# nickirk/pymes

Measured on AMD Instinct MI355X. Metric: ccsd_iteration_time, lower is better.
Workload: dtype f64

## Files before the change

include/pymes_amd.h:

```cpp
#ifndef PYMES_AMD_H
#define PYMES_AMD_H

#include <stdint.h>

#ifdef __cplusplus
extern "C" {
#endif

typedef struct pymes_ctx pymes_ctx;

#define PYMES_NOCC_MAX_FUSED 90
#define PYMES_NOCC_MAX_LAMBDA 88
#define PYMES_NOCC_MAX_BRA_DRESS 80

const char* pymes_last_error(void);
const char* pymes_backend(void);
int pymes_ctx_create(pymes_ctx** out, int device, int no, int nv, uint64_t workspace_bytes );
int pymes_ctx_destroy(pymes_ctx* ctx);
int pymes_ctx_set_stream(pymes_ctx* ctx, void* hip_stream);
int pymes_ctx_sync(pymes_ctx* ctx);
int pymes_ctx_workspace(pymes_ctx* ctx, uint64_t* capacity_bytes, uint64_t* high_water_bytes);

int pymes_malloc(pymes_ctx* ctx, uint64_t bytes, void** dev_ptr);
int pymes_free(pymes_ctx* ctx, void* dev_ptr);
// ... 14 lines not shown
int pymes_download(pymes_ctx* ctx, void* dst_host, const void* src_dev, uint64_t bytes);
int pymes_copy(pymes_ctx* ctx, void* dst_dev, const void* src_dev, uint64_t bytes);
int pymes_memset_zero(pymes_ctx* ctx, void* dst_dev, uint64_t bytes);

int pymes_contract(pymes_ctx* ctx, double alpha,
                   const double* A_dev, const char* la, const int64_t* dimA, const int64_t* strideA,
                   const double* B_dev, const char* lb, const int64_t* dimB, const int64_t* strideB,
                   double beta, double* C_dev, const char* lc, const int64_t* dimC, const int64_t* strideC,
                   const char* batch);
int pymes_permute(pymes_ctx* ctx, double alpha, const double* in_dev, const char* li, const int64_t* dim_in,
                  const int64_t* stride_in, double beta, double* out_dev, const char* lo,
                  const int64_t* stride_out);
int pymes_dgemm(pymes_ctx* ctx, int64_t M, int64_t N, int64_t K, double alpha, const double* A_dev, int64_t a_sm,
                int64_t a_sk, const double* B_dev, int64_t b_sk, int64_t b_sn, double beta, double* C_dev,
                int64_t ldc);

int pymes_set_V_pqrs(pymes_ctx* ctx, const double* V, int on_device, const int64_t* strides);
int pymes_set_V_block(pymes_ctx* ctx, const char* name, const double* data, int64_t n_elements, int on_device,
                      const int64_t* strides);
int pymes_V_exchange_asymmetry(pymes_ctx* ctx, double* out_host);
int pymes_exchange_asymmetry(pymes_ctx* ctx, const double* A_dev, const double* B_dev, const int64_t* dims,
                             double* out_host);
int pymes_set_V_from_factors(pymes_ctx* ctx, const double* B_host, int naux);
int pymes_set_integral_shard(pymes_ctx* ctx, int rank, int world);
int pymes_set_integral_direct(pymes_ctx* ctx, int64_t chunk_bytes);
int pymes_direct_info(pymes_ctx* ctx, int64_t* info);
int pymes_direct_rows(pymes_ctx* ctx, int64_t r0, int64_t r1, const double** vp, const double** vm, int64_t* ldp, int64_t* ldm);
int pymes_integral_bytes(pymes_ctx* ctx, int64_t* bytes);
int pymes_shard_rows_ptr(pymes_ctx* ctx, const double** vp, const double** vm, int64_t* row0, int64_t* row1, int64_t* ldp,
                         int64_t* ldm);
// ... 299 lines not shown
```

pymes_amd/_lib.py:

```python
import ctypes as C
import os

import numpy as np

_HERE = os.path.dirname(os.path.abspath(__file__))
DEFAULT_PATH = os.environ.get("PYMES_AMD_LIBRARY") or os.path.join(_HERE, "lib", "libpymes_amd.so")

c_double_p = C.POINTER(C.c_double)
c_i64_p = C.POINTER(C.c_int64)


class ShardBuffers(C.Structure):
    _fields_ = [(k, C.c_void_p) for k in ("ETd", "ETx", "L", "QK", "Tall", "W", "Xvv", "P", "R1", "S")]

c_pp = C.POINTER(C.c_void_p)

RESPONSE_HIST = 32
RESPONSE_DOTS = 2 * (RESPONSE_HIST + 2)


class ResponseSystem(C.Structure):
    _fields_ = ([(k, C.c_void_p * 2) for k in ("x", "r", "p", "ap", "pn")]
                + [(k, (C.c_void_p * 2) * RESPONSE_HIST) for k in ("hp", "hq")]
                + [("g", (C.c_double * 2) * RESPONSE_HIST), ("alpha", C.c_double * 2), ("z", C.c_double * 2), ("inv", C.c_double),
# ... 20 lines not shown
    "pymes_graph_abort": (C.c_int, [C.c_void_p]),
    "pymes_graph_launch": (C.c_int, [C.c_void_p, C.c_void_p]),
    "pymes_graph_destroy": (C.c_int, [C.c_void_p, C.c_void_p]),
    "pymes_upload": (C.c_int, [C.c_void_p, C.c_void_p, C.c_void_p, C.c_uint64]),
    "pymes_download": (C.c_int, [C.c_void_p, C.c_void_p, C.c_void_p, C.c_uint64]),
    "pymes_copy": (C.c_int, [C.c_void_p, C.c_void_p, C.c_void_p, C.c_uint64]),
    "pymes_memset_zero": (C.c_int, [C.c_void_p, C.c_void_p, C.c_uint64]),
    "pymes_contract": (C.c_int, [C.c_void_p, C.c_double,
                                 C.c_void_p, C.c_char_p, c_i64_p, c_i64_p,
                                 C.c_void_p, C.c_char_p, c_i64_p, c_i64_p,
                                 C.c_double, C.c_void_p, C.c_char_p, c_i64_p, c_i64_p, C.c_char_p]),
    "pymes_permute": (C.c_int, [C.c_void_p, C.c_double, C.c_void_p, C.c_char_p, c_i64_p, c_i64_p,
                                C.c_double, C.c_void_p, C.c_char_p, c_i64_p]),
    "pymes_dgemm": (C.c_int, [C.c_void_p, C.c_int64, C.c_int64, C.c_int64, C.c_double, C.c_void_p, C.c_int64,
                              C.c_int64, C.c_void_p, C.c_int64, C.c_int64, C.c_double, C.c_void_p, C.c_int64]),
    "pymes_set_V_pqrs": (C.c_int, [C.c_void_p, C.c_void_p, C.c_int, c_i64_p]),
    "pymes_set_V_block": (C.c_int, [C.c_void_p, C.c_char_p, C.c_void_p, C.c_int64, C.c_int, c_i64_p]),
    "pymes_V_exchange_asymmetry": (C.c_int, [C.c_void_p, c_double_p]),
    "pymes_exchange_asymmetry": (C.c_int, [C.c_void_p, C.c_void_p, C.c_void_p, c_i64_p, c_double_p]),
    "pymes_set_V_from_factors": (C.c_int, [C.c_void_p, C.c_void_p, C.c_int]),
    "pymes_V_block_ptr": (C.c_int, [C.c_void_p, C.c_char_p, C.c_int, c_pp, c_i64_p]),
    "pymes_set_integral_shard": (C.c_int, [C.c_void_p, C.c_int, C.c_int]),
    "pymes_integral_bytes": (C.c_int, [C.c_void_p, c_i64_p]),
    "pymes_set_integral_direct": (C.c_int, [C.c_void_p, C.c_int64]),
    "pymes_direct_info": (C.c_int, [C.c_void_p, c_i64_p]),
    "pymes_direct_rows": (C.c_int, [C.c_void_p, C.c_int64, C.c_int64, c_pp, c_pp, c_i64_p, c_i64_p]),
    "pymes_shard_rows_ptr": (C.c_int, [C.c_void_p, c_pp, c_pp, c_i64_p, c_i64_p, c_i64_p, c_i64_p]),
    "pymes_ccsd_t_triples": (C.c_int, [C.c_void_p, c_i64_p]),
    "pymes_ccsd_t": (C.c_int, [C.c_void_p, C.c_void_p, C.c_void_p, C.c_void_p, C.c_int64, C.c_int64, C.c_void_p,
                               c_double_p]),
# ... 215 lines not shown
```

pymes_amd/csrc/capi.cpp:

```cpp
#include <chrono>
#include <cstdio>
#include <cstring>
#include <exception>
#include <algorithm>
#include <mutex>
#include <set>
#include <string>
#include <vector>

#include "../../include/pymes_amd.h"
#include "diis_small.h"
#include "engine.h"
#include "eom.h"
#include "fcidump.h"
#include "packed.h"

using pymes::Engine;
using pymes::TView;

struct pymes_ctx {
    Engine* e;
};
struct pymes_eom {
    pymes::EomSigma* s;
// ... 238 lines not shown
        if (static_cast<int>(std::strlen(lo)) != r) throw pymes::Error("permute: label strings differ in length");
        int64_t dout[6];
        for (int i = 0; i < r; ++i) {
            const char* f = std::strchr(li, lo[i]);
            if (!f) throw pymes::Error("permute: output label missing from input");
            dout[i] = dim_in[f - li];
        }
        need_forward(stride_out, r, "stride_out");
        TView vout = pymes::make_view(out, r, dout, stride_out);
        need(out, "out");
        E(ctx).permute(alpha, vin, li, beta, vout, lo);
    });
}
int pymes_dgemm(pymes_ctx* ctx, int64_t M, int64_t N, int64_t K, double alpha, const double* A, int64_t a_sm,
                int64_t a_sk, const double* B, int64_t b_sk, int64_t b_sn, double beta, double* C, int64_t ldc) {
    return guarded([&] {
        Engine& e = Eq(ctx);
        dev::Gemm g{};
        g.M = M; g.N = N; g.K = K; g.alpha = alpha; g.beta = beta;
        g.A = A; g.a_sm = a_sm; g.a_sk = a_sk;
        g.B = B; g.b_sk = b_sk; g.b_sn = b_sn;
        g.C = C; g.ldc = ldc;
        g.nb1 = g.nb2 = 1;
        g.splitk_ws = e.splitk_ws();
        g.splitk_ws_doubles = e.splitk_ws_doubles();
        dev::gemm(g, e.stream);
        e.stats.gemm_calls++;
        e.stats.gemm_flops += 2.0 * double(M) * double(N) * double(K);
    });
}

int pymes_set_V_pqrs(pymes_ctx* ctx, const double* V, int on_device, const int64_t* strides) {
    return guarded([&] {
        need(V, "V");
        if (on_device) need_forward(strides, 4, "strides");
        E(ctx).set_V_full(V, on_device != 0, strides);
    });
// ... 1280 lines not shown
```

pymes_amd/csrc/kernels.hip:

```cpp
#include <hip/hip_runtime.h>
#include <type_traits>

#include <algorithm>
#include <atomic>
#include <chrono>
#include <cmath>
#include <cstdio>
#include <cstdlib>
#include <cstring>
#include <mutex>
#include <stdexcept>
#include <string>
#include <vector>

#include "../../include/pymes_amd.h"
#include "device_api.h"
#include "diis_small.h"
#include "device_util.h"
#include "launch.h"

namespace {

constexpr int kThreads = 256;
constexpr int BK = 16;
// ... 3 lines not shown
    const double* B;
    double* C;
    const double* Cin;
    long a_ld, b_ld, ldc;
    int M, N, K;
    int Mc, Nc;
    double alpha, beta;
    int tiles_m, tiles_n;
    int nsplit, kchunk;
    long tile_begin;
    long nb2;
    long a_b1, a_b2, b_b1, b_b2, c_b1, c_b2;
    double* ws;
    long whole = 0, tail = 0;
    int mixed = 0;
};

__device__ __forceinline__ long xcd_remap(long b, long nblk) {
    const long q = nblk >> 3, r = nblk & 7;
    const long xcd = b & 7, pos = b >> 3;
    return (xcd < r ? xcd * (q + 1) : r * (q + 1) + (xcd - r) * q) + pos;
}

template <int BM, int BN, bool AKC, bool BKC, int VEC, bool STREAM = false>
__device__ __forceinline__ void dgemm_body(const GemmK& g, const long bid) {
    extern __shared__ __attribute__((aligned(16))) double smem[];
    constexpr int WM = BM / 2, WN = BN / 2;
    constexpr int FM = WM / 16, FN = WN / 16;
    constexpr int A_PITCH = AKC ? (BK + 2) : (BM + 16);
    constexpr int A_ROWS = AKC ? BM : BK;
    constexpr int A_TILE = A_PITCH * A_ROWS;
    constexpr int B_PITCH = BKC ? (BK + 2) : (BN + 16);
    constexpr int B_ROWS = BKC ? BN : BK;
    constexpr int B_TILE = B_PITCH * B_ROWS;
    constexpr int LA = BM * BK / (kThreads * VEC);
    constexpr int LB = BN * BK / (kThreads * VEC);
// ... 291 lines not shown
    const unsigned lo = __builtin_amdgcn_readfirstlane((unsigned)v);
    const unsigned hi = __builtin_amdgcn_readfirstlane((unsigned)(v >> 32));
    return (const char*)(((unsigned long long)hi << 32) | lo);
}

__device__ __forceinline__ void glds16_su(const char* base_uniform, unsigned voff, unsigned lds_addr_uniform) {
    asm volatile("s_mov_b32 m0, %2\n\ts_nop 0\n\tglobal_load_lds_dwordx4 %0, %1"
                 :
                 : "v"(voff), "s"(base_uniform), "s"(lds_addr_uniform)
                 : "memory", "m0");
}
__device__ __forceinline__ unsigned lds_addr_of(const double* p) {
    return (unsigned)(unsigned long long)(const __attribute__((address_space(3))) void*)p;
}

template <bool AKC, bool BKC>
__device__ __forceinline__ void dgemm_glds_tile(const GemmK& g, const long gt, const int kbeg, const int kend,
                                                double* __restrict__ Wpart) {
    extern __shared__ __attribute__((aligned(16))) double smem[];
    constexpr int BM = 128, BN = 128, WM = 64, WN = 64, FM = 4, FN = 4;
    constexpr int A_PITCH = AKC ? BK : (BM + 16);
    constexpr int A_TILE = AKC ? BM * BK : BK * A_PITCH;
    constexpr int B_PITCH = BKC ? BK : (BN + 16);
    constexpr int B_TILE = BKC ? BN * BK : BK * B_PITCH;
    double* As = smem;
    double* Bs = smem + 2 * A_TILE;

    const int tid = threadIdx.x;
    const int lane = tid & 63, wave = __builtin_amdgcn_readfirstlane(tid >> 6);
    const int wm = wave >> 1, wn = wave & 1;
    const int l15 = lane & 15, l4 = lane >> 4;

    const int tiles = g.tiles_m * g.tiles_n;
    const long z = gt / tiles;
    const int t = (int)(gt - z * tiles);
    constexpr int GROUP = 8;
    const int group_sz = GROUP * g.tiles_n;
    const int grp = t / group_sz;
    const int first_m = grp * GROUP;
    const int gm = min(g.tiles_m - first_m, GROUP);
    const int tin = t - grp * group_sz;
    const int tm = uni(first_m + tin % gm);
    const int tn = uni(tin / gm);
    const long z1 = z / g.nb2, z2 = z - z1 * g.nb2;
    const int m0 = tm * BM, n0 = tn * BN;
    const int nkt = (kend - kbeg + BK - 1) / BK;
    const int nfull = (kend - kbeg) / BK;

    const char* ua = uni_ptr(g.A + z1 * g.a_b1 + z2 * g.a_b2 + (AKC ? (long)m0 * g.a_ld + kbeg : (long)kbeg * g.a_ld + m0));
    const char* ub = uni_ptr(g.B + z1 * g.b_b1 + z2 * g.b_b2 + (BKC ? (long)n0 * g.b_ld + kbeg : (long)kbeg * g.b_ld + n0));
    unsigned ao[4], bo[4];
#pragma unroll
    for (int j = 0; j < 4; ++j) {
        if (AKC) {
            const int row = wave * 32 + (lane >> 3) + 8 * j;
            const int cg = (lane & 7) ^ ((row >> 1) & 7);
            ao[j] = ((unsigned)(min(m0 + row, g.M - 1) - m0) * (unsigned)g.a_ld + cg * 2) * 8u;
        } else {
// ... 3 lines not shown
            const int row = wave * 32 + (lane >> 3) + 8 * j;
            const int cg = (lane & 7) ^ ((row >> 1) & 7);
            bo[j] = ((unsigned)(min(n0 + row, g.N - 1) - n0) * (unsigned)g.b_ld + cg * 2) * 8u;
        } else {
            bo[j] = ((unsigned)(wave * 4 + j) * (unsigned)g.b_ld + (unsigned)(min(n0 + 2 * lane, g.Nc - 2) - n0)) * 8u;
        }
    }
    const long a_kstep = 8 * (AKC ? (long)BK : (long)BK * g.a_ld);
    const long b_kstep = 8 * (BKC ? (long)BK : (long)BK * g.b_ld);
    const int a_dst = AKC ? wave * 32 * BK : wave * 4 * A_PITCH;
    const int b_dst = BKC ? wave * 32 * BK : wave * 4 * B_PITCH;
    constexpr int A_DSTEP = AKC ? 8 * BK : A_PITCH;
    constexpr int B_DSTEP = BKC ? 8 * BK : B_PITCH;

    const unsigned a_lds = uni((int)lds_addr_of(As + a_dst)), b_lds = uni((int)lds_addr_of(Bs + b_dst));
    auto stage_dma = [&](int buf) {
        const unsigned as = a_lds + buf * (A_TILE * 8), bs = b_lds + buf * (B_TILE * 8);
#pragma unroll
        for (int j = 0; j < 4; ++j) glds16_su(ua, ao[j], as + j * (A_DSTEP * 8));
#pragma unroll
        for (int j = 0; j < 4; ++j) glds16_su(ub, bo[j], bs + j * (B_DSTEP * 8));
        ua += a_kstep;
        ub += b_kstep;
    };
    auto stage_tail = [&](int buf, int k0) {
        const unsigned as = a_lds + buf * (A_TILE * 8), bs = b_lds + buf * (B_TILE * 8);
        const v2d zero = {0.0, 0.0};
#pragma unroll
        for (int j = 0; j < 4; ++j) {
            bool in_a, in_b;
            if (AKC) {
                const int row = wave * 32 + (lane >> 3) + 8 * j;
                in_a = k0 + (((lane & 7) ^ ((row >> 1) & 7)) << 1) < kend;
            } else {
                in_a = k0 + wave * 4 + j < kend;
            }
            if (BKC) {
                const int row = wave * 32 + (lane >> 3) + 8 * j;
                in_b = k0 + (((lane & 7) ^ ((row >> 1) & 7)) << 1) < kend;
            } else {
                in_b = k0 + wave * 4 + j < kend;
            }
            if (in_a) glds16_su(ua, ao[j], as + j * (A_DSTEP * 8));
            else *reinterpret_cast<v2d*>(As + buf * A_TILE + a_dst + j * A_DSTEP + 2 * lane) = zero;
            if (in_b) glds16_su(ub, bo[j], bs + j * (B_DSTEP * 8));
            else *reinterpret_cast<v2d*>(Bs + buf * B_TILE + b_dst + j * B_DSTEP + 2 * lane) = zero;
        }
    };

    v4d acc[FM][FN];
#pragma unroll
    for (int i = 0; i < FM; ++i)
#pragma unroll
        for (int j = 0; j < FN; ++j) acc[i][j] = v4d{0.0, 0.0, 0.0, 0.0};

    const int fsw = (l15 >> 1) & 7;
    int a_koff[4], b_koff[4];
#pragma unroll
    for (int kk = 0; kk < 4; ++kk) {
        const int sw = (((2 * kk + (l4 >> 1)) ^ fsw) << 1) + (l4 & 1);
        a_koff[kk] = AKC ? (wm * WM + l15) * BK + sw : (kk * 4 + l4) * A_PITCH + wm * WM + l15;
        b_koff[kk] = BKC ? (wn * WN + l15) * BK + sw : (kk * 4 + l4) * B_PITCH + wn * WN + l15;
    }
    constexpr int A_FSTEP = AKC ? 16 * BK : 16;
    constexpr int B_FSTEP = BKC ? 16 * BK : 16;

    double a[2][FM], b[2][FN];
    auto read_frags = [&](const double* as, const double* bs, int kk, double (&ra_)[FM], double (&rb_)[FN]) {
#pragma unroll
        for (int i = 0; i < FM; ++i) ra_[i] = as[a_koff[kk] + i * A_FSTEP];
#pragma unroll
        for (int j = 0; j < FN; ++j) rb_[j] = bs[b_koff[kk] + j * B_FSTEP];
    };
    auto mfma_step = [&](const double (&ra_)[FM], const double (&rb_)[FN]) {
#pragma unroll
        for (int i = 0; i < FM; ++i)
#pragma unroll
            for (int j = 0; j < FN; ++j)
                acc[i][j] = __builtin_amdgcn_mfma_f64_16x16x4f64(ra_[i], rb_[j], acc[i][j], 0, 0, 0);
    };
    auto landed = [&]() {
        asm volatile("s_waitcnt vmcnt(0) lgkmcnt(0)" ::: "memory");
        __builtin_amdgcn_s_barrier();
    };
    auto ktile = [&](auto curc, int next, int k_next) {
        constexpr int cur = decltype(curc)::value;
        if (next == 1) stage_dma(cur ^ 1);
        else if (next == 2) stage_tail(cur ^ 1, k_next);
        const double* as = As + cur * A_TILE;
        const double* bs = Bs + cur * B_TILE;
        read_frags(as, bs, 1, a[1], b[1]);
        mfma_step(a[0], b[0]);
        read_frags(as, bs, 2, a[0], b[0]);
        mfma_step(a[1], b[1]);
        read_frags(as, bs, 3, a[1], b[1]);
        mfma_step(a[0], b[0]);
        landed();
        if (next) read_frags(As + (cur ^ 1) * A_TILE, Bs + (cur ^ 1) * B_TILE, 0, a[0], b[0]);
        mfma_step(a[1], b[1]);
    };
    const std::integral_constant<int, 0> buf0;
    const std::integral_constant<int, 1> buf1;

    if (nkt > 0) {
        if (nfull > 0) stage_dma(0);
        else stage_tail(0, kbeg);
        landed();
        read_frags(As, Bs, 0, a[0], b[0]);
        int kt = 0;
        for (; kt + 2 < nfull; kt += 2) {
            ktile(buf0, 1, 0);
            ktile(buf1, 1, 0);
        }
        auto next_of = [&](int t) { return t + 1 < nfull ? 1 : (t + 1 < nkt ? 2 : 0); };
        ktile(buf0, next_of(kt), kbeg + (kt + 1) * BK);
        if (kt + 1 < nkt) {
            ktile(buf1, next_of(kt + 1), kbeg + (kt + 2) * BK);
            if (kt + 2 < nkt) ktile(buf0, 0, 0);
        }
    } else {
        landed();
    }

    if (Wpart) {
        double* __restrict__ W = Wpart;
#pragma unroll
        for (int i = 0; i < FM; ++i)
#pragma unroll
            for (int j = 0; j < FN; ++j)
#pragma unroll
                for (int r = 0; r < 4; ++r)
                    W[(wm * WM + i * 16 + l4 + 4 * r) * BN + wn * WN + j * 16 + l15] = acc[i][j][r];
        return;
    }
    double* C = g.C + z1 * g.c_b1 + z2 * g.c_b2;
    const double* Cin = g.Cin + z1 * g.c_b1 + z2 * g.c_b2;
    const long ldc = g.ldc;
    const double alpha = g.alpha, beta = g.beta;
#pragma unroll
    for (int i = 0; i < FM; ++i) {
#pragma unroll
        for (int j = 0; j < FN; ++j) {
            const int n = n0 + wn * WN + j * 16 + l15;
#pragma unroll
            for (int r = 0; r < 4; ++r) {
                const int m = m0 + wm * WM + i * 16 + l4 + 4 * r;
                if (m < g.M && n < g.N) {
// ... 26 lines not shown
        cut = g.nsplit > 1;
    }
    const int kbeg = cut ? ks * g.kchunk : 0;
    const int kend = cut ? min(g.K, kbeg + g.kchunk) : g.K;
    dgemm_glds_tile<AKC, BKC>(g, g.tile_begin + lt, kbeg, kend,
                              cut ? g.ws + ((lt - (g.mixed ? g.whole : 0)) * g.nsplit + ks) * 16384L : nullptr);
}

template <bool AKC, bool BKC>
__global__ void __launch_bounds__(kThreads, 2) dgemm_glds_kernel(const GemmK g) {
    const long b = blockIdx.x;
    const long id = !g.mixed ? xcd_remap(b, gridDim.x)
                             : (b < g.whole ? xcd_remap(b, g.whole) : g.whole + xcd_remap(b - g.whole, (long)gridDim.x - g.whole));
    dgemm_glds_body<AKC, BKC>(g, id);
}
__global__ void __launch_bounds__(kThreads, 2) dgemm_glds_group_kernel(const GroupK grp) {
    const long gb = xcd_remap(blockIdx.x, gridDim.x);
    int it = 0;
    while (it + 1 < grp.n && gb >= grp.blk_end[it]) ++it;
    dgemm_glds_body<true, false>(grp.g[it], gb - (it ? grp.blk_end[it - 1] : 0));
}

__device__ __forceinline__ void splitk_reduce_body(const GemmK& g, const int BM, const int BN, const long lt, const int piece) {
    const int tiles = g.tiles_m * g.tiles_n;
    const long gt = g.tile_begin + lt;
    const long z = gt / tiles;
    const int t = (int)(gt - z * tiles);
    constexpr int GROUP = 8;
    const int group_sz = GROUP * g.tiles_n;
    const int grp = t / group_sz;
    const int first_m = grp * GROUP;
    const int gm = min(g.tiles_m - first_m, GROUP);
    const int tin = t - grp * group_sz;
    const int tm = first_m + tin % gm;
    const int tn = tin / gm;
    const long z1 = z / g.nb2, z2 = z - z1 * g.nb2;
    double* C = g.C + z1 * g.c_b1 + z2 * g.c_b2;
    const double* Cin = g.Cin + z1 * g.c_b1 + z2 * g.c_b2;
    const double* __restrict__ W = g.ws + lt * g.nsplit * (long)(BM * BN);
    const int e = piece * 256 + threadIdx.x;
    const int r = e / BN, c = e - r * BN;
    const int m = tm * BM + r, n = tn * BN + c;
    if (m >= g.M || n >= g.N) return;
    const long st = (long)BM * BN;
    double s0 = 0.0, s1 = 0.0, s2 = 0.0, s3 = 0.0;
    int k = 0;
    for (; k + 16 <= g.nsplit; k += 16) {
        double w[16];
#pragma unroll
        for (int q = 0; q < 16; ++q) w[q] = W[(long)(k + q) * st + e];
#pragma unroll
        for (int q = 0; q < 16; q += 4) { s0 += w[q]; s1 += w[q + 1]; s2 += w[q + 2]; s3 += w[q + 3]; }
    }
    for (; k + 4 <= g.nsplit; k += 4) {
        s0 += W[(long)k * st + e];
        s1 += W[(long)(k + 1) * st + e];
        s2 += W[(long)(k + 2) * st + e];
        s3 += W[(long)(k + 3) * st + e];
    }
// ... 2778 lines not shown
    constexpr int B_T = (BKC ? (BK + 2) * BN : (BN + 16) * BK);
    constexpr size_t lds = (size_t)(STREAM ? 1 : 2) * (A_T + B_T) * sizeof(double);
    allow_dynamic_lds<dgemm_kernel<BM, BN, AKC, BKC, VEC, STREAM>>(lds);
    launch_kernel(dgemm_kernel<BM, BN, AKC, BKC, VEC, STREAM>, dim3((unsigned)nblocks), dim3(kThreads), lds, st, k);
}

template <bool AKC, bool BKC>
void launch_gemm_glds(const GemmK& k, long nblocks, hipStream_t st) {
    constexpr int A_T = AKC ? 128 * BK : BK * (128 + 16);
    constexpr int B_T = BKC ? 128 * BK : BK * (128 + 16);
    constexpr size_t lds = (size_t)2 * (A_T + B_T) * sizeof(double);
    allow_dynamic_lds<dgemm_glds_kernel<AKC, BKC>>(lds);
    launch_kernel(dgemm_glds_kernel<AKC, BKC>, dim3((unsigned)nblocks), dim3(kThreads), lds, st, k);
}

inline long dma_min_k() { return 384L; }

inline long cut_k(long ktiles, long want, GemmK* k = nullptr) {
    const long kt_per = (ktiles + want - 1) / want;
    const long nsplit = std::max<long>(1, (ktiles + kt_per - 1) / std::max<long>(kt_per, 1));
    if (k) { k->kchunk = (int)std::max<long>(kt_per * BK, BK); k->nsplit = (int)nsplit; }
    return nsplit;
}

struct DmaPlan { long whole, tail; int s; };
inline DmaPlan plan_dma(long tiles, long ktiles, long ws_tiles) {
    const long whole = (tiles / 256) * 256, tail = tiles - whole;
    DmaPlan best{tiles, 0, 1};
    const long max_cuts = std::max<long>(1, ktiles / (dma_min_k() / BK));
    if (tail > 0) {
// ... 84 lines not shown
    const dev::Gemm& g = p.g;
    GemmK k;
    k.A = g.A; k.B = g.B; k.C = g.C;
    k.Cin = g.Cin ? g.Cin : g.C;
    k.a_ld = p.a_ld; k.b_ld = p.b_ld; k.ldc = g.ldc;
    k.M = (int)g.M; k.N = (int)g.N; k.K = (int)g.K;
    k.Mc = p.Mc; k.Nc = p.Nc;
    k.alpha = g.alpha; k.beta = g.beta;
    k.tiles_m = (int)((g.M + BM - 1) / BM);
    k.tiles_n = (int)((g.N + BN - 1) / BN);
    k.tile_begin = 0;
    k.nb2 = g.nb2;
    k.a_b1 = g.a_b1; k.a_b2 = g.a_b2; k.b_b1 = g.b_b1; k.b_b2 = g.b_b2; k.c_b1 = g.c_b1; k.c_b2 = g.c_b2;
    k.ws = nullptr;
    return k;
}

struct TailSplit { long main_tiles, tail_tiles; int split; };
inline TailSplit plan_tail(long tiles, long ktiles, long slots, long min_kt, long ws_tiles) {
    const long rem = tiles % slots;
    if (ktiles < 16 || rem == 0) return {tiles, 0, 1};
    long best = 1;
    double best_cost = 1.0;
    long smax = std::min<long>(512, std::max<long>(8, 2048 / rem));
    smax = std::min<long>(smax, ktiles / min_kt);
    smax = std::min<long>(smax, ws_tiles / rem);
    for (long sp = 2; sp <= smax; ++sp) {
        const double cost = (double)((rem * sp + slots - 1) / slots) / (double)sp + 1e-5 * sp;
        if (cost < best_cost - 1e-9) { best_cost = cost; best = sp; }
    }
// ... 518 lines not shown
    if (BM == 64 && BN == 64) {
        if (g.N <= 32) BN = 32;
        else if (g.M <= 32) BM = 32;
    }
    GemmK k = make_gemmk(p, BM, BN);
    const long tiles = (long)k.tiles_m * k.tiles_n * p.nbatch;
    if (tiles > 0x7fffffffL) throw std::runtime_error("gemm: grid too large");

    const long slots = (BM <= 64 && BN <= 64) ? 1024 : 256;
    const long ws_tiles = g.splitk_ws ? g.splitk_ws_doubles / ((long)BM * BN) : 0;
    const bool dma_ok = BM == 128 && BN == 128 && p.vec == 2 && g.K >= dma_min_k() &&
                        (p.akc ? 128 : 16) * k.a_ld * 8 + 4096 < (1L << 32) &&
                        (p.bkc ? 128 : 16) * k.b_ld * 8 + 4096 < (1L << 32);
    DmaPlan plan{tiles, 0, 1};
    if (dma_ok) plan = plan_dma(tiles, ktiles, ws_tiles);
    const TailSplit ts = dma_ok ? TailSplit{tiles, 0, 1} : plan_tail(tiles, ktiles, slots, (BM == 128 && BN == 128) ? 16 : 8, ws_tiles);

    ProfSpan span(st);
    bool used_dma = false;
    int n_kernels = 0;
    g_stream64 = stream && BM <= 64 && BN <= 64;
    auto launch = [&](long tile_begin, long ntiles, int nsplit) {
        k.tile_begin = tile_begin;
        k.ws = cut_k(ktiles, nsplit, &k) > 1 ? g.splitk_ws : nullptr;
        const long nblocks = ntiles * k.nsplit;
        ++n_kernels;
        if (BM == 128 && BN == 128) dispatch_layout<128, 128>(k, p.akc, p.bkc, p.vec, nblocks, st);
        else if (BM == 128 && BN == 64) dispatch_layout<128, 64>(k, p.akc, p.bkc, p.vec, nblocks, st);
        else if (BM == 64 && BN == 128) dispatch_layout<64, 128>(k, p.akc, p.bkc, p.vec, nblocks, st);
        else if (BM == 64 && BN == 32) dispatch_layout<64, 32>(k, p.akc, p.bkc, p.vec, nblocks, st);
        else if (BM == 32 && BN == 64) dispatch_layout<32, 64>(k, p.akc, p.bkc, p.vec, nblocks, st);
        else dispatch_layout<64, 64>(k, p.akc, p.bkc, p.vec, nblocks, st);
        if (k.nsplit > 1) {
            launch_kernel(splitk_reduce_kernel, dim3((unsigned)ntiles, (unsigned)(BM * BN / 256)), dim3(256), 0, st, k, BM, BN);
        }
        return k.nsplit;
    };
    int nsplit = 1;
    if (dma_ok) {
        if (cut_k(ktiles, plan.s, &k) == 1) { plan.whole = tiles; plan.tail = 0; }
        k.mixed = 1;
        k.whole = plan.whole;
        k.tail = plan.tail;
        k.ws = plan.tail > 0 ? g.splitk_ws : nullptr;
        const long nblocks = plan.whole + plan.tail * k.nsplit;
        if (nblocks > 0x7fffffffL) throw std::runtime_error("gemm: grid too large");
        if (p.akc && p.bkc) launch_gemm_glds<true, true>(k, nblocks, st);
        else if (p.akc) launch_gemm_glds<true, false>(k, nblocks, st);
        else if (p.bkc) launch_gemm_glds<false, true>(k, nblocks, st);
        else launch_gemm_glds<false, false>(k, nblocks, st);
        used_dma = true;
        n_kernels = 1;
        if (plan.tail > 0) {
            GemmK r = k;
            r.tile_begin = plan.whole;
            r.mixed = 0;
            launch_kernel(splitk_reduce_kernel, dim3((unsigned)plan.tail, 64u), dim3(256), 0, st, r, 128, 128);
            nsplit = -k.nsplit;
        }
    } else {
        nsplit = ts.main_tiles > 0 ? launch(0, ts.main_tiles, 1) : 1;
        if (ts.tail_tiles > 0) nsplit = -launch(ts.main_tiles, ts.tail_tiles, ts.split);
    }
    if (g_prof.on) {
        char buf[256];
        int len = snprintf(buf, sizeof buf, "M=%ld N=%ld K=%ld batch=%ld tile=%dx%d%s akc=%d bkc=%d vec=%d dma=%d split=%d flops=%.4e",
                           (long)g.M, (long)g.N, (long)g.K, (long)p.nbatch, BM, BN, g_stream64 ? "s" : "", (int)p.akc,
                           (int)p.bkc, p.vec, (int)used_dma, nsplit, p.flops);
        if (used_dma && len > 0 && len < (int)sizeof buf)
            snprintf(buf + len, sizeof buf - len, " plan=%ld+%ld/%d", plan.whole, plan.tail, plan.tail ? k.nsplit : 1);
        span.finish(p.flops, used_dma ? 1 : 0, n_kernels, buf);
    }
}

void gemv_batch_begin() {
    g_gemv_batch.active = true;
    g_gemv_batch.tab.n = 0;
    g_gemv_batch.ws_used = 0;
}
void gemv_batch_end() {
    gemv_batch_flush();
    g_gemv_batch.active = false;
}

void permute(const Permute& p, stream_t s) {
// ... 941 lines not shown
```

pymes_amd/device.py:

```python
import ctypes as C
import weakref

import numpy as np

from . import _lib
from ._lib import PymesError, i64_array, ptr_array

BLOCK_NAMES = ("abci", "iabj", "iajk", "aijk", "klij", "aibj", "ijak", "abic",
               "iajb", "abcd", "iabc", "aijb", "ijka", "aibc", "ijab", "abij")


def pattern_of(name):
    return sum((1 << (3 - p)) for p, ch in enumerate(name) if ch in "abcd")


class DeviceArray:

    def __init__(self, ctx, ptr, shape, owned=True, keepalive=None):
        self.ctx, self.ptr, self.shape = ctx, int(ptr), tuple(int(s) for s in shape)
        self._owned, self._keep = owned, keepalive
        self.size = int(np.prod(self.shape)) if self.shape else 1

    @property
    def nbytes(self):
# ... 209 lines not shown
                      C.c_void_p(B.ptr), lb.encode(), i64_array(B.shape), None,
                      float(beta), C.c_void_p(out.ptr), lc.encode(), i64_array(out.shape), None, batch.encode())
        return out

    def permute(self, spec, A, out=None, alpha=1.0, beta=0.0, in_view=None):
        li, lo = spec.replace(" ", "").split("->")
        dims = tuple(A.shape) if in_view is None else tuple(int(d) for d in in_view[0])
        shape_o = tuple(dims[li.index(ch)] for ch in lo)
        if out is None:
            out = self.empty(shape_o)
            beta = 0.0
        self.lib.call("pymes_permute", self.handle, float(alpha), C.c_void_p(A.ptr), li.encode(), i64_array(dims),
                      None if in_view is None else i64_array(in_view[1]), float(beta), C.c_void_p(out.ptr), lo.encode(), None)
        return out

    def dgemm(self, M, N, K, alpha, A, a_sm, a_sk, B, b_sk, b_sn, beta, Cmat, ldc):
        self.lib.call("pymes_dgemm", self.handle, M, N, K, float(alpha), C.c_void_p(A.ptr), a_sm, a_sk,
                      C.c_void_p(B.ptr), b_sk, b_sn, float(beta), C.c_void_p(Cmat.ptr), ldc)

    def set_V_pqrs(self, V):
        if isinstance(V, DeviceArray):
            self.lib.call("pymes_set_V_pqrs", self.handle, C.c_void_p(V.ptr), 1, None)
        else:
            V = np.ascontiguousarray(V, dtype=np.float64)
            if V.shape != (self.n,) * 4:
                raise ValueError(f"V_pqrs must have shape {(self.n,) * 4}")
            self.lib.call("pymes_set_V_pqrs", self.handle, _lib.host_ptr(V), 0, None)

    def set_V_block(self, name, data):
        want = self.block_shape(name)
        if tuple(data.shape) != want:
# ... 521 lines not shown
```

Baseline: 0.1599.

## Absorb small M/N remainders into enlarged edge tiles in DMA GEMM

Adds a 'fat' edge-tile mode to the LDS-DMA DGEMM. When M or N leaves a remainder of 1-16 past a multiple of 128, the last row or column of tiles grows to 144 instead of launching a mostly empty extra tile. Extra 16-wide strips are staged through LDS and computed with additional MFMAs on selected waves, and the split-K reduce and workspace slots are sized to match. It also adds a dgemm entry point that takes a separate C input. The mode is gated by tile count (at least 512), an A K-contiguous / B N-contiguous layout and an environment variable. The risks are a larger LDS footprint and an uneven load across the waves of edge blocks.

```diff
diff --git a/include/pymes_amd.h b/include/pymes_amd.h
--- a/include/pymes_amd.h
+++ b/include/pymes_amd.h
@@ -52,6 +52,9 @@
 int pymes_dgemm(pymes_ctx* ctx, int64_t M, int64_t N, int64_t K, double alpha, const double* A_dev, int64_t a_sm,
                 int64_t a_sk, const double* B_dev, int64_t b_sk, int64_t b_sn, double beta, double* C_dev,
                 int64_t ldc);
+int pymes_dgemm_cin(pymes_ctx* ctx, int64_t M, int64_t N, int64_t K, double alpha, const double* A_dev, int64_t a_sm,
+                    int64_t a_sk, const double* B_dev, int64_t b_sk, int64_t b_sn, double beta, const double* Cin_dev,
+                    double* C_dev, int64_t ldc);
 
 int pymes_set_V_pqrs(pymes_ctx* ctx, const double* V, int on_device, const int64_t* strides);
 int pymes_set_V_block(pymes_ctx* ctx, const char* name, const double* data, int64_t n_elements, int on_device,
diff --git a/pymes_amd/_lib.py b/pymes_amd/_lib.py
--- a/pymes_amd/_lib.py
+++ b/pymes_amd/_lib.py
@@ -58,6 +58,8 @@
                                 C.c_double, C.c_void_p, C.c_char_p, c_i64_p]),
     "pymes_dgemm": (C.c_int, [C.c_void_p, C.c_int64, C.c_int64, C.c_int64, C.c_double, C.c_void_p, C.c_int64,
                               C.c_int64, C.c_void_p, C.c_int64, C.c_int64, C.c_double, C.c_void_p, C.c_int64]),
+    "pymes_dgemm_cin": (C.c_int, [C.c_void_p, C.c_int64, C.c_int64, C.c_int64, C.c_double, C.c_void_p, C.c_int64,
+                                  C.c_int64, C.c_void_p, C.c_int64, C.c_int64, C.c_double, C.c_void_p, C.c_void_p, C.c_int64]),
     "pymes_set_V_pqrs": (C.c_int, [C.c_void_p, C.c_void_p, C.c_int, c_i64_p]),
     "pymes_set_V_block": (C.c_int, [C.c_void_p, C.c_char_p, C.c_void_p, C.c_int64, C.c_int, c_i64_p]),
     "pymes_V_exchange_asymmetry": (C.c_int, [C.c_void_p, c_double_p]),
diff --git a/pymes_amd/csrc/capi.cpp b/pymes_amd/csrc/capi.cpp
--- a/pymes_amd/csrc/capi.cpp
+++ b/pymes_amd/csrc/capi.cpp
@@ -276,6 +276,11 @@
 }
 int pymes_dgemm(pymes_ctx* ctx, int64_t M, int64_t N, int64_t K, double alpha, const double* A, int64_t a_sm,
                 int64_t a_sk, const double* B, int64_t b_sk, int64_t b_sn, double beta, double* C, int64_t ldc) {
+    return pymes_dgemm_cin(ctx, M, N, K, alpha, A, a_sm, a_sk, B, b_sk, b_sn, beta, nullptr, C, ldc);
+}
+int pymes_dgemm_cin(pymes_ctx* ctx, int64_t M, int64_t N, int64_t K, double alpha, const double* A, int64_t a_sm,
+                    int64_t a_sk, const double* B, int64_t b_sk, int64_t b_sn, double beta, const double* Cin, double* C,
+                    int64_t ldc) {
     return guarded([&] {
         Engine& e = Eq(ctx);
         dev::Gemm g{};
@@ -283,6 +288,7 @@
         g.A = A; g.a_sm = a_sm; g.a_sk = a_sk;
         g.B = B; g.b_sk = b_sk; g.b_sn = b_sn;
         g.C = C; g.ldc = ldc;
+        g.Cin = beta != 0.0 ? Cin : nullptr;
         g.nb1 = g.nb2 = 1;
         g.splitk_ws = e.splitk_ws();
         g.splitk_ws_doubles = e.splitk_ws_doubles();
diff --git a/pymes_amd/csrc/kernels.hip b/pymes_amd/csrc/kernels.hip
--- a/pymes_amd/csrc/kernels.hip
+++ b/pymes_amd/csrc/kernels.hip
@@ -41,12 +41,40 @@
     double* ws;
     long whole = 0, tail = 0;
     int mixed = 0;
+    int fat = 0;
 };
+__host__ __device__ inline long glds_fat_slot(int fat) { return (long)((fat & 1) ? 144 : 128) * ((fat & 2) ? 144 : 128); }
 
 __device__ __forceinline__ long xcd_remap(long b, long nblk) {
     const long q = nblk >> 3, r = nblk & 7;
     const long xcd = b & 7, pos = b >> 3;
     return (xcd < r ? xcd * (q + 1) : r * (q + 1) + (xcd - r) * q) + pos;
+}
+
+__device__ __forceinline__ void gemm_tile_rc(const GemmK& g, const long gt, int& tm, int& tn) {
+    const int tiles = g.tiles_m * g.tiles_n;
+    const int t = (int)(gt - (gt / tiles) * tiles);
+    int rows = g.tiles_m, cols = g.tiles_n;
+    if (g.fat) {
+        rows -= g.fat & 1;
+        cols -= (g.fat >> 1) & 1;
+        int e = t - rows * cols;
+        if (e >= 0) {
+            if (g.fat & 1) {
+                if (e < cols) { tm = rows; tn = e; return; }
+                e -= cols;
+            }
+            tm = e;
+            tn = cols;
+            return;
+        }
+    }
+    const int group_sz = 8 * cols;
+    const int grp = t / group_sz;
+    const int gm = min(rows - grp * 8, 8);
+    const int tin = t - grp * group_sz;
+    tm = grp * 8 + tin % gm;
+    tn = tin / gm;
 }
 
 template <int BM, int BN, bool AKC, bool BKC, int VEC, bool STREAM = false>
@@ -368,25 +396,34 @@
     return (unsigned)(unsigned long long)(const __attribute__((address_space(3))) void*)p;
 }
 
-template <bool AKC, bool BKC>
+template <bool AKC, bool BKC, int FAT = 0, int SEL = 0, bool FAT_ORDER = (FAT != 0)>
 __device__ __forceinline__ void dgemm_glds_tile(const GemmK& g, const long gt, const int kbeg, const int kend,
                                                 double* __restrict__ Wpart) {
+    static_assert(FAT == 0 || (AKC && !BKC), "fat tiles: A K-contiguous, B N-contiguous");
     extern __shared__ __attribute__((aligned(16))) double smem[];
     constexpr int BM = 128, BN = 128, WM = 64, WN = 64, FM = 4, FN = 4;
     constexpr int A_PITCH = AKC ? BK : (BM + 16);
     constexpr int A_TILE = AKC ? BM * BK : BK * A_PITCH;
     constexpr int B_PITCH = BKC ? BK : (BN + 16);
     constexpr int B_TILE = BKC ? BN * BK : BK * B_PITCH;
+    constexpr bool FATM = (FAT & 1) != 0, FATN = (FAT & 2) != 0;
+    constexpr int XM = 2 * (SEL & 1);
+    constexpr int XN = SEL & 2;
+    constexpr bool CORNER = FAT == 3 && SEL == 3;
+    constexpr int STRIP = 16 * BK;
+    constexpr int WPITCH = FATN ? BN + 16 : BN;
     double* As = smem;
-    double* Bs = smem + 2 * A_TILE;
+    double* AsS = smem + 2 * A_TILE;
+    double* Bs = smem + 2 * A_TILE + (FAT != 0 ? 2 * STRIP : 0);
+    double* BsS = Bs + 2 * B_TILE;
 
     const int tid = threadIdx.x;
     const int lane = tid & 63, wave = __builtin_amdgcn_readfirstlane(tid >> 6);
-    const int wm = wave >> 1, wn = wave & 1;
+    const int wm = FATM ? (SEL & 1) : wave >> 1, wn = FATN ? (SEL >> 1) : wave & 1;
     const int l15 = lane & 15, l4 = lane >> 4;
 
     const int tiles = g.tiles_m * g.tiles_n;
-    const long z = gt / tiles;
+    const long z = FAT != 0 ? (long)uni((int)(gt / tiles)) : gt / tiles;
     const int t = (int)(gt - z * tiles);
     constexpr int GROUP = 8;
     const int group_sz = GROUP * g.tiles_n;
@@ -394,8 +431,10 @@
     const int first_m = grp * GROUP;
     const int gm = min(g.tiles_m - first_m, GROUP);
     const int tin = t - grp * group_sz;
-    const int tm = uni(first_m + tin % gm);
-    const int tn = uni(tin / gm);
+    int tm_v = first_m + tin % gm, tn_v = tin / gm;
+    if constexpr (FAT_ORDER) gemm_tile_rc(g, gt, tm_v, tn_v);
+    const int tm = uni(tm_v);
+    const int tn = uni(tn_v);
     const long z1 = z / g.nb2, z2 = z - z1 * g.nb2;
     const int m0 = tm * BM, n0 = tn * BN;
     const int nkt = (kend - kbeg + BK - 1) / BK;
@@ -429,12 +468,31 @@
     constexpr int B_DSTEP = BKC ? 8 * BK : B_PITCH;
 
     const unsigned a_lds = uni((int)lds_addr_of(As + a_dst)), b_lds = uni((int)lds_addr_of(Bs + b_dst));
+    constexpr bool A_STRIP = FATM && !(SEL & 1), B_STRIP = FATN && (SEL & 2);
+    unsigned aso = 0, bso = 0, as_lds = 0, bs_lds = 0;
+    if constexpr (A_STRIP) {
+        const int row = wn * 8 + (lane >> 3);
+        const int cg = (lane & 7) ^ ((row >> 1) & 7);
+        aso = ((unsigned)(min(m0 + BM + row, g.M - 1) - m0) * (unsigned)g.a_ld + cg * 2) * 8u;
+        as_lds = uni((int)lds_addr_of(AsS + wn * (STRIP / 2)));
+    }
+    if constexpr (B_STRIP) {
+        bso = ((unsigned)(wm * 8 + (lane >> 3)) * (unsigned)g.b_ld + (unsigned)(min(n0 + BN + 2 * (lane & 7), g.Nc - 2) - n0)) * 8u;
+        bs_lds = uni((int)lds_addr_of(BsS + wm * (STRIP / 2)));
+    }
+    const long a_jstep = FATM ? 16L * 8 * g.a_ld : 0, b_jstep = FATN ? 8L * g.b_ld : 0;
+    auto ua_of = [&](int j) { return FATM ? ua + (j >> 1) * a_jstep : ua; };
+    auto ao_of = [&](int j) { return FATM ? ao[j & 1] : ao[j]; };
+    auto ub_of = [&](int j) { return FATN ? ub + j * b_jstep : ub; };
+    auto bo_of = [&](int j) { return FATN ? bo[0] : bo[j]; };
     auto stage_dma = [&](int buf) {
         const unsigned as = a_lds + buf * (A_TILE * 8), bs = b_lds + buf * (B_TILE * 8);
 #pragma unroll
-        for (int j = 0; j < 4; ++j) glds16_su(ua, ao[j], as + j * (A_DSTEP * 8));
-#pragma unroll
-        for (int j = 0; j < 4; ++j) glds16_su(ub, bo[j], bs + j * (B_DSTEP * 8));
+        for (int j = 0; j < 4; ++j) glds16_su(ua_of(j), ao_of(j), as + j * (A_DSTEP * 8));
+#pragma unroll
+        for (int j = 0; j < 4; ++j) glds16_su(ub_of(j), bo_of(j), bs + j * (B_DSTEP * 8));
+        if constexpr (A_STRIP) glds16_su(ua, aso, as_lds + buf * (STRIP * 8));
+        if constexpr (B_STRIP) glds16_su(ub, bso, bs_lds + buf * (STRIP * 8));
         ua += a_kstep;
         ub += b_kstep;
     };
@@ -456,10 +514,19 @@
             } else {
                 in_b = k0 + wave * 4 + j < kend;
             }
-            if (in_a) glds16_su(ua, ao[j], as + j * (A_DSTEP * 8));
+            if (in_a) glds16_su(ua_of(j), ao_of(j), as + j * (A_DSTEP * 8));
             else *reinterpret_cast<v2d*>(As + buf * A_TILE + a_dst + j * A_DSTEP + 2 * lane) = zero;
-            if (in_b) glds16_su(ub, bo[j], bs + j * (B_DSTEP * 8));
+            if (in_b) glds16_su(ub_of(j), bo_of(j), bs + j * (B_DSTEP * 8));
             else *reinterpret_cast<v2d*>(Bs + buf * B_TILE + b_dst + j * B_DSTEP + 2 * lane) = zero;
+        }
+        if constexpr (A_STRIP) {
+            const int row = wn * 8 + (lane >> 3);
+            if (k0 + (((lane & 7) ^ ((row >> 1) & 7)) << 1) < kend) glds16_su(ua, aso, as_lds + buf * (STRIP * 8));
+            else *reinterpret_cast<v2d*>(AsS + buf * STRIP + wn * (STRIP / 2) + 2 * lane) = zero;
+        }
+        if constexpr (B_STRIP) {
+            if (k0 + wm * 8 + (lane >> 3) < kend) glds16_su(ub, bso, bs_lds + buf * (STRIP * 8));
+            else *reinterpret_cast<v2d*>(BsS + buf * STRIP + wm * (STRIP / 2) + 2 * lane) = zero;
         }
     };
 
@@ -479,6 +546,25 @@
     }
     constexpr int A_FSTEP = AKC ? 16 * BK : 16;
     constexpr int B_FSTEP = BKC ? 16 * BK : 16;
+
+    v4d accm[2], accn[2], accc;
+    double ea[2], eb[2];
+    if constexpr (FAT != 0) accm[0] = accm[1] = accn[0] = accn[1] = accc = v4d{0.0, 0.0, 0.0, 0.0};
+    auto read_strips = [&](int buf, int kk, int x) {
+        if constexpr (FATM) ea[x] = AsS[buf * STRIP + a_koff[kk] - (SEL & 1) * WM * BK];
+        if constexpr (FATN) eb[x] = BsS[buf * STRIP + kk * 64 + lane];
+    };
+    auto mfma_strips = [&](const double (&ra_)[FM], const double (&rb_)[FN], int x) {
+        if constexpr (FATM) {
+            accm[0] = __builtin_amdgcn_mfma_f64_16x16x4f64(ea[x], rb_[XM], accm[0], 0, 0, 0);
+            accm[1] = __builtin_amdgcn_mfma_f64_16x16x4f64(ea[x], rb_[XM + 1], accm[1], 0, 0, 0);
+        }
+        if constexpr (FATN) {
+            accn[0] = __builtin_amdgcn_mfma_f64_16x16x4f64(ra_[XN], eb[x], accn[0], 0, 0, 0);
+            accn[1] = __builtin_amdgcn_mfma_f64_16x16x4f64(ra_[XN + 1], eb[x], accn[1], 0, 0, 0);
+        }
+        if constexpr (CORNER) accc = __builtin_amdgcn_mfma_f64_16x16x4f64(ea[x], eb[x], accc, 0, 0, 0);
+    };
 
     double a[2][FM], b[2][FN];
     auto read_frags = [&](const double* as, const double* bs, int kk, double (&ra_)[FM], double (&rb_)[FN]) {
@@ -505,14 +591,24 @@
         const double* as = As + cur * A_TILE;
         const double* bs = Bs + cur * B_TILE;
         read_frags(as, bs, 1, a[1], b[1]);
+        read_strips(cur, 1, 1);
         mfma_step(a[0], b[0]);
+        mfma_strips(a[0], b[0], 0);
         read_frags(as, bs, 2, a[0], b[0]);
+        read_strips(cur, 2, 0);
         mfma_step(a[1], b[1]);
+        mfma_strips(a[1], b[1], 1);
         read_frags(as, bs, 3, a[1], b[1]);
+        read_strips(cur, 3, 1);
         mfma_step(a[0], b[0]);
+        mfma_strips(a[0], b[0], 0);
         landed();
-        if (next) read_frags(As + (cur ^ 1) * A_TILE, Bs + (cur ^ 1) * B_TILE, 0, a[0], b[0]);
+        if (next) {
+            read_frags(As + (cur ^ 1) * A_TILE, Bs + (cur ^ 1) * B_TILE, 0, a[0], b[0]);
+            read_strips(cur ^ 1, 0, 0);
+        }
         mfma_step(a[1], b[1]);
+        mfma_strips(a[1], b[1], 1);
     };
     const std::integral_constant<int, 0> buf0;
     const std::integral_constant<int, 1> buf1;
@@ -522,6 +618,7 @@
         else stage_tail(0, kbeg);
         landed();
         read_frags(As, Bs, 0, a[0], b[0]);
+        read_strips(0, 0, 0);
         int kt = 0;
         for (; kt + 2 < nfull; kt += 2) {
             ktile(buf0, 1, 0);
@@ -537,6 +634,25 @@
         landed();
     }
 
+    if constexpr (FAT != 0) {
+        auto emit = [&](const v4d& v, int mb, int nb) {
+#pragma unroll
+            for (int r = 0; r < 4; ++r) {
+                const int mt = mb * 16 + l4 + 4 * r, nt = nb * 16 + l15;
+                if (Wpart) {
+                    Wpart[mt * WPITCH + nt] = v[r];
+                } else if (m0 + mt < g.M && n0 + nt < g.N) {
+                    const long off = z1 * g.c_b1 + z2 * g.c_b2 + (long)(m0 + mt) * g.ldc + (n0 + nt);
+                    double o = g.alpha * v[r];
+                    if (g.beta != 0.0) o += g.beta * g.Cin[off];
+                    g.C[off] = o;
+                }
+            }
+        };
+        if constexpr (FATM) { emit(accm[0], 8, 4 * wn + XM); emit(accm[1], 8, 4 * wn + XM + 1); }
+        if constexpr (FATN) { emit(accn[0], 4 * wm + XN, 8); emit(accn[1], 4 * wm + XN + 1, 8); }
+        if constexpr (CORNER) emit(accc, 8, 8);
+    }
     if (Wpart) {
         double* __restrict__ W = Wpart;
 #pragma unroll
@@ -545,7 +661,7 @@
             for (int j = 0; j < FN; ++j)
 #pragma unroll
                 for (int r = 0; r < 4; ++r)
-                    W[(wm * WM + i * 16 + l4 + 4 * r) * BN + wn * WN + j * 16 + l15] = acc[i][j][r];
+                    W[(wm * WM + i * 16 + l4 + 4 * r) * WPITCH + wn * WN + j * 16 + l15] = acc[i][j][r];
         return;
     }
     double* C = g.C + z1 * g.c_b1 + z2 * g.c_b2;
@@ -602,6 +718,55 @@
                              : (b < g.whole ? xcd_remap(b, g.whole) : g.whole + xcd_remap(b - g.whole, (long)gridDim.x - g.whole));
     dgemm_glds_body<AKC, BKC>(g, id);
 }
+
+__global__ void __launch_bounds__(kThreads, 2) dgemm_glds_fat_kernel(const GemmK g) {
+    const long b = blockIdx.x;
+    const long bid = !g.mixed ? xcd_remap(b, gridDim.x)
+                              : (b < g.whole ? xcd_remap(b, g.whole) : g.whole + xcd_remap(b - g.whole, (long)gridDim.x - g.whole));
+    long lt;
+    int ks;
+    bool cut;
+    if (g.mixed) {
+        if (bid < g.whole) { lt = bid; ks = 0; cut = false; }
+        else {
+            const long r = bid - g.whole;
+            ks = uni((int)(r / g.tail));
+            lt = g.whole + (r - (long)ks * g.tail);
+            cut = true;
+        }
+    } else {
+        lt = bid / g.nsplit;
+        ks = uni((int)(bid - lt * g.nsplit));
+        cut = g.nsplit > 1;
+    }
+    const int kbeg = cut ? ks * g.kchunk : 0;
+    const int kend = cut ? min(g.K, kbeg + g.kchunk) : g.K;
+    double* W = cut ? g.ws + ((lt - (g.mixed ? g.whole : 0)) * g.nsplit + ks) * glds_fat_slot(g.fat) : nullptr;
+    const long gt = g.tile_begin + lt;
+    int tm, tn;
+    gemm_tile_rc(g, gt, tm, tn);
+    const int kind = uni((((g.fat & 1) && tm == g.tiles_m - 1) ? 1 : 0) | (((g.fat & 2) && tn == g.tiles_n - 1) ? 2 : 0));
+    const int wave = __builtin_amdgcn_readfirstlane(threadIdx.x >> 6);
+    const int wm = wave >> 1, wn = wave & 1;
+    switch (kind) {
+        case 0: dgemm_glds_tile<true, false, 0, 0, true>(g, gt, kbeg, kend, W); break;
+        case 1:
+            if (wm) dgemm_glds_tile<true, false, 1, 1>(g, gt, kbeg, kend, W);
+            else dgemm_glds_tile<true, false, 1, 0>(g, gt, kbeg, kend, W);
+            break;
+        case 2:
+            if (wn) dgemm_glds_tile<true, false, 2, 2>(g, gt, kbeg, kend, W);
+            else dgemm_glds_tile<true, false, 2, 0>(g, gt, kbeg, kend, W);
+            break;
+        default:
+            switch (wave) {
+                case 0: dgemm_glds_tile<true, false, 3, 0>(g, gt, kbeg, kend, W); break;
+                case 1: dgemm_glds_tile<true, false, 3, 2>(g, gt, kbeg, kend, W); break;
+                case 2: dgemm_glds_tile<true, false, 3, 1>(g, gt, kbeg, kend, W); break;
+                default: dgemm_glds_tile<true, false, 3, 3>(g, gt, kbeg, kend, W); break;
+            }
+    }
+}
 __global__ void __launch_bounds__(kThreads, 2) dgemm_glds_group_kernel(const GroupK grp) {
     const long gb = xcd_remap(blockIdx.x, gridDim.x);
     int it = 0;
@@ -620,17 +785,21 @@
     const int first_m = grp * GROUP;
     const int gm = min(g.tiles_m - first_m, GROUP);
     const int tin = t - grp * group_sz;
-    const int tm = first_m + tin % gm;
-    const int tn = tin / gm;
+    int tm = first_m + tin % gm;
+    int tn = tin / gm;
+    if (g.fat) gemm_tile_rc(g, gt, tm, tn);
     const long z1 = z / g.nb2, z2 = z - z1 * g.nb2;
     double* C = g.C + z1 * g.c_b1 + z2 * g.c_b2;
     const double* Cin = g.Cin + z1 * g.c_b1 + z2 * g.c_b2;
-    const double* __restrict__ W = g.ws + lt * g.nsplit * (long)(BM * BN);
+    const int bmt = ((g.fat & 1) && tm == g.tiles_m - 1) ? BM + 16 : BM;
+    const int bnt = ((g.fat & 2) && tn == g.tiles_n - 1) ? BN + 16 : BN;
+    const long st = g.fat ? glds_fat_slot(g.fat) : (long)BM * BN;
+    const double* __restrict__ W = g.ws + lt * g.nsplit * st;
     const int e = piece * 256 + threadIdx.x;
-    const int r = e / BN, c = e - r * BN;
+    if (e >= bmt * bnt) return;
+    const int r = e / bnt, c = e - r * bnt;
     const int m = tm * BM + r, n = tn * BN + c;
     if (m >= g.M || n >= g.N) return;
-    const long st = (long)BM * BN;
     double s0 = 0.0, s1 = 0.0, s2 = 0.0, s3 = 0.0;
     int k = 0;
     for (; k + 16 <= g.nsplit; k += 16) {
@@ -3439,6 +3608,12 @@
     launch_kernel(dgemm_glds_kernel<AKC, BKC>, dim3((unsigned)nblocks), dim3(kThreads), lds, st, k);
 }
 
+void launch_gemm_glds_fat(const GemmK& k, long nblocks, hipStream_t st) {
+    constexpr size_t lds = (size_t)2 * (128 * BK + BK * (128 + 16) + 2 * 16 * BK) * sizeof(double);
+    allow_dynamic_lds<dgemm_glds_fat_kernel>(lds);
+    launch_kernel(dgemm_glds_fat_kernel, dim3((unsigned)nblocks), dim3(kThreads), lds, st, k);
+}
+
 inline long dma_min_k() { return 384L; }
 
 inline long cut_k(long ktiles, long want, GemmK* k = nullptr) {
@@ -3553,6 +3728,19 @@
     k.a_b1 = g.a_b1; k.a_b2 = g.a_b2; k.b_b1 = g.b_b1; k.b_b2 = g.b_b2; k.c_b1 = g.c_b1; k.c_b2 = g.c_b2;
     k.ws = nullptr;
     return k;
+}
+
+inline int fat_edges(const GemmProduct& p, const GemmK& k, long tiles) {
+    if (!p.akc || p.bkc) return 0;
+    const char* e = getenv("PYMES_GEMM_FAT");
+    const int mode = e && *e ? atoi(e) : -1;
+    if (mode == 0) return 0;
+    if (mode != 1 && (tiles < 512 || getenv("PYMES_GEMM_PLAN"))) return 0;
+    int fat = 0;
+    const int rm = k.M % 128, rn = k.N % 128;
+    if (k.M > 128 && rm >= 1 && rm <= 16 && 144 * k.a_ld * 8 + 4096 < (1L << 32)) fat |= 1;
+    if (k.N > 128 && rn >= 1 && rn <= 16) fat |= 2;
+    return fat;
 }
 
 struct TailSplit { long main_tiles, tail_tiles; int split; };
@@ -4101,6 +4289,17 @@
                         (p.bkc ? 128 : 16) * k.b_ld * 8 + 4096 < (1L << 32);
     DmaPlan plan{tiles, 0, 1};
     if (dma_ok) plan = plan_dma(tiles, ktiles, ws_tiles);
+    if (const int fat = dma_ok ? fat_edges(p, k, tiles) : 0) {
+        GemmK kf = k;
+        kf.fat = fat;
+        if (fat & 1) --kf.tiles_m;
+        if (fat & 2) --kf.tiles_n;
+        const long tiles_f = (long)kf.tiles_m * kf.tiles_n * p.nbatch;
+        const long ws_tiles_f = g.splitk_ws ? g.splitk_ws_doubles / glds_fat_slot(fat) : 0;
+        const DmaPlan pf = plan_dma(tiles_f, ktiles, ws_tiles_f), pu = plan_dma(tiles_f, ktiles, 1L << 40);
+        if (pf.whole == pu.whole && pf.s == pu.s) { k = kf; plan = pf; }
+    }
+    const long tiles_run = (long)k.tiles_m * k.tiles_n * p.nbatch;
     const TailSplit ts = dma_ok ? TailSplit{tiles, 0, 1} : plan_tail(tiles, ktiles, slots, (BM == 128 && BN == 128) ? 16 : 8, ws_tiles);
 
     ProfSpan span(st);
@@ -4125,14 +4324,15 @@
     };
     int nsplit = 1;
     if (dma_ok) {
-        if (cut_k(ktiles, plan.s, &k) == 1) { plan.whole = tiles; plan.tail = 0; }
+        if (cut_k(ktiles, plan.s, &k) == 1) { plan.whole = tiles_run; plan.tail = 0; }
         k.mixed = 1;
         k.whole = plan.whole;
         k.tail = plan.tail;
         k.ws = plan.tail > 0 ? g.splitk_ws : nullptr;
         const long nblocks = plan.whole + plan.tail * k.nsplit;
         if (nblocks > 0x7fffffffL) throw std::runtime_error("gemm: grid too large");
-        if (p.akc && p.bkc) launch_gemm_glds<true, true>(k, nblocks, st);
+        if (k.fat) launch_gemm_glds_fat(k, nblocks, st);
+        else if (p.akc && p.bkc) launch_gemm_glds<true, true>(k, nblocks, st);
         else if (p.akc) launch_gemm_glds<true, false>(k, nblocks, st);
         else if (p.bkc) launch_gemm_glds<false, true>(k, nblocks, st);
         else launch_gemm_glds<false, false>(k, nblocks, st);
@@ -4142,7 +4342,8 @@
             GemmK r = k;
             r.tile_begin = plan.whole;
             r.mixed = 0;
-            launch_kernel(splitk_reduce_kernel, dim3((unsigned)plan.tail, 64u), dim3(256), 0, st, r, 128, 128);
+            const unsigned pieces = (unsigned)((k.fat ? glds_fat_slot(k.fat) : 16384L) / 256);
+            launch_kernel(splitk_reduce_kernel, dim3((unsigned)plan.tail, pieces), dim3(256), 0, st, r, 128, 128);
             nsplit = -k.nsplit;
         }
     } else {
@@ -4155,7 +4356,8 @@
                            (long)g.M, (long)g.N, (long)g.K, (long)p.nbatch, BM, BN, g_stream64 ? "s" : "", (int)p.akc,
                            (int)p.bkc, p.vec, (int)used_dma, nsplit, p.flops);
         if (used_dma && len > 0 && len < (int)sizeof buf)
-            snprintf(buf + len, sizeof buf - len, " plan=%ld+%ld/%d", plan.whole, plan.tail, plan.tail ? k.nsplit : 1);
+            snprintf(buf + len, sizeof buf - len, "%s plan=%ld+%ld/%d", k.fat == 3 ? " fat=mn" : k.fat == 2 ? " fat=n" : k.fat ? " fat=m" : "",
+                     plan.whole, plan.tail, plan.tail ? k.nsplit : 1);
         span.finish(p.flops, used_dma ? 1 : 0, n_kernels, buf);
     }
 }
diff --git a/pymes_amd/device.py b/pymes_amd/device.py
--- a/pymes_amd/device.py
+++ b/pymes_amd/device.py
@@ -247,7 +247,11 @@
                       None if in_view is None else i64_array(in_view[1]), float(beta), C.c_void_p(out.ptr), lo.encode(), None)
         return out
 
-    def dgemm(self, M, N, K, alpha, A, a_sm, a_sk, B, b_sk, b_sn, beta, Cmat, ldc):
+    def dgemm(self, M, N, K, alpha, A, a_sm, a_sk, B, b_sk, b_sn, beta, Cmat, ldc, Cin=None):
+        if Cin is not None:
+            self.lib.call("pymes_dgemm_cin", self.handle, M, N, K, float(alpha), C.c_void_p(A.ptr), a_sm, a_sk,
+                          C.c_void_p(B.ptr), b_sk, b_sn, float(beta), C.c_void_p(Cin.ptr), C.c_void_p(Cmat.ptr), ldc)
+            return
         self.lib.call("pymes_dgemm", self.handle, M, N, K, float(alpha), C.c_void_p(A.ptr), a_sm, a_sk,
                       C.c_void_p(B.ptr), b_sk, b_sn, float(beta), C.c_void_p(Cmat.ptr), ldc)
 
```

New measurement: 0.1575, median of 6. 1.5% less time.
